# Dunni3/keypoint-diffusion

Measured on AMD Instinct MI355X. Metric: denoising steps/sec, higher is better.
Workload: dtype f32; 1 GPU; egnn_all_atom dynamics (6 EGNN layers, hidden 256, update_kp_feat; fixed receptor encoder), batch of 64 synthetic 300-atom pockets / 25-atom ligands per GPU, T=500, seeded random-init weights, every step taken from the t=T ligand state; batch_per_gpu=64, n_rec=300, n_lig=25, parallelism=dp1

## Files before the change

keypoint-diffusion_amd/csrc/egnn.hip:

```cpp
#include <string.h>

#include <map>
#include <set>
#include <string>
#include <vector>

#include "egnn_kernels.h"
#include "egnn_wide.h"
#include "mfma_core.h"

using namespace kpd;

namespace {

struct LayerW {
    float *wp_e[4], *wx_e[4], *b_e[4], *wr_e[4], *watt[4];
    float *wp_c[4], *wx_c[4], *b_c[4], *wr_c[4], *w3[4];
    void *wh_e[4], *wh_c[4];
    void *chh_p[2][NSLOT];
    void *wh_a[2], *wh_b[2], *wh_2[2];
    float *wp_p[2][NSLOT], *wx_p[2][NSLOT], *b_p[2][NSLOT];
    float *ch_p[2][NSLOT], *wcol_p[2][NSLOT];
    float *wp_a[2], *wx_a[2], *wp_b[2], *wx_b[2], *b0[2], *wp_2[2], *wx_2[2], *b2[2], *ln_w[2], *ln_b[2];
};
// ... 517 lines not shown
                                       void *stream) {
    KPD_REQUIRE(m && bt && t_dev && eps_h && eps_x, KPD_ERR_INVALID, "null argument");
    KPD_REQUIRE(m->wide || m->committed, KPD_ERR_STATE, "kpd_egnn_forward before kpd_egnn_commit");
    KPD_REQUIRE(bt->B >= 1 && bt->n_lig >= 1 && bt->n_kp >= 1, KPD_ERR_INVALID, "empty batch (B=%d n_lig=%d n_kp=%d)", bt->B, bt->n_lig, bt->n_kp);
    KPD_REQUIRE(!m->cfg.update_kp_feat || bt->n_kk == 0 || (bt->kk_src && bt->kk_dst), KPD_ERR_INVALID, "kk edges missing");
    KPD_REQUIRE(bt->kk_rowptr, KPD_ERR_INVALID, "kk_rowptr missing");
    if (m->wide) return wide_forward(m->wide, bt, t_dev, eps_h, eps_x, static_cast<hipStream_t>(stream));
    KPD_REQUIRE(bt->B <= m->cap_B && bt->n_lig <= m->cap_lig && bt->n_kp <= m->cap_kp && bt->n_kk <= m->cap_kk &&
                    bt->max_lig <= m->cap_maxlig && bt->max_kp <= m->cap_maxkp,
                KPD_ERR_CAPACITY, "batch (B=%d lig=%d kp=%d kk=%d maxlig=%d maxkp=%d) exceeds reserved workspace (%d %d %d %d %d %d)",
                bt->B, bt->n_lig, bt->n_kp, bt->n_kk, bt->max_lig, bt->max_kp, m->cap_B, m->cap_lig, m->cap_kp, m->cap_kk,
                m->cap_maxlig, m->cap_maxkp);
    hipStream_t st = static_cast<hipStream_t>(stream);
    const kpd_egnn_config &c = m->cfg;

    KPD_HIP(hipMemcpyAsync(m->x[NT_LIG], bt->lig_x, (size_t)bt->n_lig * 12, hipMemcpyDeviceToDevice, st));
    KPD_HIP(hipMemcpyAsync(m->x[NT_KP], bt->kp_x, (size_t)bt->n_kp * 12, hipMemcpyDeviceToDevice, st));
    KPD_TRY(launch_node_graph_index(bt->lig_ptr, bt->B, bt->n_lig, m->bidx[NT_LIG], st));
    KPD_TRY(launch_node_graph_index(bt->kp_ptr, bt->B, bt->n_kp, m->bidx[NT_KP], st));
    KPD_TRY(launch_lig_graph(bt, c.ll_cutoff, c.ll_k, c.kl_cutoff, c.kl_k, &m->lg, m->ll_deg, m->ll_off, m->kl_off, m->kl_pg, st));
    const int tr = TM;
    const int active = c.update_kp_feat ? 0xF : 0x3;
    const bool prune = c.update_kp_feat && m->prune_last;
    const int active_last = prune ? 0x3 : active;
    KPD_TRY(launch_egnn_meta(m->lg.counts, bt->n_kk, active, active_last, bt->lig_ptr, bt->kp_ptr, m->lg.ll_per_graph,
                             bt->kk_rowptr, bt->B, m->kl_off, c.message_norm, c.update_kp_feat, m->meta, m->z[NT_LIG],
                             m->z[NT_KP], st, tr));
    KPD_TRY(launch_embed(bt->lig_h, bt->n_lig, c.atom_nf, m->le_W0, m->le_b0, 64, m->le_W1t, m->le_b1, t_dev,
                         m->bidx[NT_LIG], m->h[NT_LIG], 0, st));
    KPD_TRY(launch_embed(bt->kp_h, bt->n_kp, c.rec_nf, m->re_W0, m->re_b0, 2 * c.rec_nf, m->re_W1t, m->re_b1, t_dev,
                         m->bidx[NT_KP], m->h[NT_KP], m->rec_identity ? 1 : 0, st));
    const int n_tab = bt->B * c.rec_nf;
    const bool kp_tab = m->kp_table && m->gemm_mode == 0 && m->tab_rows > 0 && (long)bt->B * c.rec_nf <= bt->n_kp / 2;
    m->last_table = kp_tab;
    if (kp_tab) {
        KPD_REQUIRE(n_tab <= m->tab_rows, KPD_ERR_CAPACITY, "internal: %d class rows, table of %d", n_tab, m->tab_rows);
        KPD_HIP(hipMemsetD32Async(reinterpret_cast<hipDeviceptr_t>(m->kp_ok), 0x3f800000, 1, st));
        KPD_TRY(launch_kp_classify(bt->kp_h, bt->n_kp, c.rec_nf, m->bidx[NT_KP], m->rowmap, m->kp_ok, st));
        KPD_TRY(launch_embed(m->tab_in, n_tab, c.rec_nf, m->re_W0, m->re_b0, 2 * c.rec_nf, m->re_W1t, m->re_b1, t_dev, m->tab_bidx,
                             m->hT, 0, st));
    }

    const int e_kl_cap = bt->n_kp * (c.kl_k > 0 ? c.kl_k : std::min(bt->max_lig, 100));
    const int E_cap[4] = {std::max<int>((long)bt->n_lig * std::min(bt->max_lig - 1, c.ll_k > 0 ? c.ll_k : 200), 1), e_kl_cap, e_kl_cap,
                          bt->n_kk};
    int tile_cap = 0, tile_cap_last = 0;
    for (int et = 0; et < m->n_et; ++et) {
        tile_cap += cdiv(E_cap[et], tr);
        if ((active_last >> et) & 1) tile_cap_last += cdiv(E_cap[et], tr);
    }

    const int n[2] = {bt->n_lig, bt->n_kp};
    const int *esrc[4] = {m->lg.ll_src, m->lg.kl_src, m->lg.lk_src, bt->kk_src};
// ... 37 lines not shown
                    pk.n_slots[NT_LIG] = 0;
                    pk.skip_if = m->kp_ok;
                    ProjArgs &pa = pp.nt[NT_KP];
                    pa.h = m->hT; pa.n = n_tab; pa.P = m->PT;
                    KPD_TRY(launch_proj_chain(pp, st));
                    KPD_TRY(launch_proj_chain(pk, st));
                } else {
                    KPD_TRY(launch_proj_chain(pp, st));
                }
            }
        }
        EdgeArgs ea;
        memset(&ea, 0, sizeof(ea));
        const bool last = li == n_layers - 1;
        ea.meta = last ? m->meta + 16 : m->meta;
        ea.x[0] = m->x[0]; ea.x[1] = m->x[1]; ea.P[0] = m->P[0]; ea.P[1] = m->P[1];
        ea.use_tanh = c.use_tanh; ea.coords_range = c.coords_range;
        ea.tile_rows = tr;
        ea.gemm_mode = tr == TM ? m->gemm_mode : 0;
        for (int et = 0; et < 4; ++et) {
            ea.src[et] = esrc[et]; ea.dst[et] = edst[et];
            ea.src_nt[et] = kSrcNt[et]; ea.dst_nt[et] = kDstNt[et]; ea.src_slot[et] = kSrcSlot[et]; ea.dst_slot[et] = kDstSlot[et];
            ea.wr_e[et] = L.wr_e[et]; ea.wr_c[et] = L.wr_c[et];
            ea.wp_e[et] = L.wp_e[et]; ea.wx_e[et] = L.wx_e[et]; ea.b_e[et] = L.b_e[et];
            ea.wp_c[et] = L.wp_c[et]; ea.wx_c[et] = L.wx_c[et]; ea.b_c[et] = L.b_c[et];
            ea.wh_e[et] = L.wh_e[et]; ea.wh_c[et] = L.wh_c[et];
            ea.watt[et] = L.watt[et]; ea.w3[et] = L.w3[et];
            ea.hn_main[et] = m->hn_main[et]; ea.hn_cont[et] = m->hn_cont[et];
            ea.xn_main[et] = m->xn_main[et]; ea.xn_cont[et] = m->xn_cont[et];
        }
        if (kp_tab && li == 0) { ea.PT = m->PT; ea.rowmap = m->rowmap; ea.kp_ok = m->kp_ok; }
// ... 18 lines not shown
            na.wp_a = L.wp_a[nt]; na.wx_a = L.wx_a[nt]; na.wp_b = L.wp_b[nt]; na.wx_b = L.wx_b[nt]; na.b0 = L.b0[nt];
            na.wp_2 = L.wp_2[nt]; na.wx_2 = L.wx_2[nt]; na.b2 = L.b2[nt]; na.ln_w = L.ln_w[nt]; na.ln_b = L.ln_b[nt];
            na.ln_inv_n = 1.0f / (float)(c.hidden_nf + 1); na.ln_pad = (float)(HID - c.hidden_nf);
            na.wh_a = L.wh_a[nt]; na.wh_b = L.wh_b[nt]; na.wh_2 = L.wh_2[nt];
            na.norm = c.norm;
            na.tile_shift = 6;
        };
        {
            NodeLayerPair lp;
            memset(&lp, 0, sizeof(lp));
            for (int nt = 0; nt < 2; ++nt) {
                NodeLayerArgs &na = lp.nt[nt];
                na.u.n = n[nt]; na.u.h = m->h[nt];
                if (nt < m->n_upd && !(nt == NT_KP && last && prune)) {
                    fill_update(na.u, nt);
                    na.do_update = 1;
                }
                if (!na.do_update && !na.do_proj) na.u.n = 0;
            }
            lp.tiles0 = cdiv(lp.nt[0].u.n, TN);
            lp.gemm_mode = m->gemm_mode;
            KPD_TRY(launch_node_layer(lp, st));
        }
    }
    KPD_TRY(launch_decode(m->h[NT_LIG], m->x[NT_LIG], bt->lig_x, bt->n_lig, c.atom_nf, 2 * c.atom_nf, m->de_W0, m->de_b0,
                          m->de_W1, m->de_b1, eps_h, eps_x, st));
    return KPD_OK;
}

extern "C" kpd_status kpd_egnn_debug_state(kpd_egnn *m, const char *what, float *out, int64_t n_floats, void *stream) {
    KPD_REQUIRE(m && what && out, KPD_ERR_INVALID, "null argument");
    hipStream_t st = static_cast<hipStream_t>(stream);
    if (m->wide) return wide_debug_state(m->wide, what, out, n_floats, st);
    const std::string w(what);
    const float *src = nullptr;
    if (w == "h_lig") src = m->h[0];
    else if (w == "h_kp") src = m->h[1];
    else if (w == "x_lig") src = m->x[0];
    else if (w == "x_kp") src = m->x[1];
// ... 100 lines not shown
```

keypoint-diffusion_amd/csrc/egnn_kernels.h:

```cpp
#pragma once
#include "engine.h"

namespace kpd {

constexpr int NSLOT = 8;
constexpr int ATT_BIAS_AT = 260;
constexpr int BIAS_K = 260;
constexpr int ET_LL = 0, ET_KL = 1, ET_LK = 2, ET_KK = 3;
constexpr int NT_LIG = 0, NT_KP = 1;

constexpr int EDGE_LDS_BYTES = TM * SA * 4 + (TM * 2 + TM + 3 * TM + TM + 3 * TM + 4 * HS + 8 + TM) * 4;
constexpr int EDGE_KPT_LDS_BYTES = EDGE_LDS_BYTES + 2 * TM * 4;
constexpr int EDGE_H_LDS_BYTES = 64 * 280 * 2 * 2 + (TM * 2 + TM + 3 * TM + TM + 3 * TM + 2 * HS + 8) * 4 + 2 * 2 * 272 * 2;

struct ProjArgs {
    const float *h;
    int n;
    float *P;
    const float *wp[NSLOT];
    const float *wx[NSLOT];
    const float *bias[NSLOT];
    int slot[NSLOT];
    const float *chain[NSLOT];
    const float *wcol[NSLOT];
    const void *chain_h[NSLOT];
};

// ... 70 lines not shown
    float *att[4], *sc[4], *nvec[4];
    const float *dij[4];
    const float *wa[4], *w3[4];
    const float *wpT[4][2], *wxT[4][2], *wr[4][2];
    float *dv_main[4][2], *dv_cont[4][2], *dvw_main[4][2], *dvw_cont[4][2];
    float *part[2];
    int part_ld;
    int use_tanh;
    float coords_range;
};

struct NodeArgs {
    int n;
    float *h;
    float *x;
    const int *bidx;
    const float *z;
    int n_in;
    const int *rowptr[2];
    const float *hn_main[2], *hn_cont[2];
    const float *xn_main[2], *xn_cont[2];
    const float *wp_a, *wx_a, *wp_b, *wx_b, *b0;
    const float *wp_2, *wx_2, *b2;
    const void *wh_a, *wh_b, *wh_2;
    const float *ln_w, *ln_b;
    int norm;
    float ln_inv_n, ln_pad;
    int tile_shift;
};

// ... 7 lines not shown
};

struct NodeLayerPair {
    NodeLayerArgs nt[2];
    int tiles0;
    int gemm_mode;
};

constexpr int TN = 32;
constexpr int NODE_LAYER_LDS_BYTES = TN * SA * 4 + 3 * TN * 4 + 3 * HS * 4;
constexpr int NODE_H_TILE_FLOATS = 2 * TN * 280 / 2;
constexpr int NODE_H_LDS_BYTES = NODE_H_TILE_FLOATS * 4 + 3 * TN * 4;


kpd_status egnn_kernels_init();
kpd_status launch_node_graph_index(const int *ptr, int B, int n, int *bidx, hipStream_t st);
kpd_status launch_egnn_meta(const int *counts, int e_kk, int active_mask, int active_last, const int *lig_ptr, const int *kp_ptr,
                            const int *ll_per_graph, const int *kk_rowptr, int B, const int *kl_off, float message_norm,
                            int update_kp, int *meta, float *z_lig, float *z_kp, hipStream_t st, int tile_rows = TM);
kpd_status launch_embed(const float *in, int n, int fin, const float *W0, const float *b0, int hid, const float *W1t,
                        const float *b1, const float *t, const int *bidx, float *out, int identity, hipStream_t st);
kpd_status launch_kp_classify(const float *kp_h, int n, int fin, const int *bidx, int *rowmap, int *ok, hipStream_t st);
kpd_status launch_decode(const float *h, const float *x, const float *x0, int n, int atom_nf, int hid, const float *W0,
                         const float *b0, const float *W1, const float *b1, float *eps_h, float *eps_x, hipStream_t st);
kpd_status launch_egnn_edge(const EdgeArgs &a, int tile_cap, hipStream_t st);
kpd_status launch_egnn_edge_train(const EdgeTrainArgs &a, int tile_cap, hipStream_t st);
struct EdgePiecesSumArgs {
    const float *hn_main[4], *hn_cont[4], *xn_main[4], *xn_cont[4];
    const int *rowptr[4];
    int live[4], dst_nt[4];
    const float *zinv[2];
    int n[2];
    float *hn[2], *xn[2];
};
kpd_status launch_edge_pieces_sum(const EdgePiecesSumArgs &a, hipStream_t st);
kpd_status launch_edge_train_pack(const EdgePackTab &t, hipStream_t st);
kpd_status launch_egnn_edge_bwd(const EdgeBwdArgs &a, int tile_cap, hipStream_t st);
// ... 15 lines not shown
```

keypoint-diffusion_amd/csrc/egnn_kernels.hip:

```cpp
#include <stdlib.h>

#include <algorithm>

#include "egnn_kernels.h"
#include "mfma_core.h"

namespace kpd {

__global__ void k_node_graph_index(const int *__restrict__ ptr, int B, int n, int *__restrict__ bidx) {
    const int i = blockIdx.x * blockDim.x + threadIdx.x;
    if (i >= n) return;
    int lo = 0, hi = B;
    while (hi - lo > 1) {
        const int mid = (lo + hi) >> 1;
        if (ptr[mid] <= i) lo = mid; else hi = mid;
    }
    bidx[i] = lo;
}

__global__ void k_kp_classify(const float *__restrict__ kp_h, int n, int fin, const int *__restrict__ bidx, int *__restrict__ rowmap,
                              int *__restrict__ ok) {
    const int v = blockIdx.x * blockDim.x + threadIdx.x;
    if (v >= n) return;
    const unsigned *row = reinterpret_cast<const unsigned *>(kp_h) + (size_t)v * fin;
    int ones = 0, other = 0, c = 0;
    for (int k = 0; k < fin; ++k) {
        const unsigned u = row[k];
        if (u == 0x3f800000u) { ++ones; c = k; }
        else if (u != 0u) other = 1;
    }
    rowmap[v] = bidx[v] * fin + c;
    if (ones != 1 || other) *ok = 0;
}

__global__ void k_egnn_meta(const int *__restrict__ counts, int e_kk, int active_mask, int active_last, const int *__restrict__ lig_ptr,
                            const int *__restrict__ kp_ptr, const int *__restrict__ ll_per_graph,
                            const int *__restrict__ kk_rowptr, int B, const int *__restrict__ kl_off, float message_norm,
                            int update_kp, int tile_rows, int *__restrict__ meta, float *__restrict__ z_lig, float *__restrict__ z_kp) {
    if (blockIdx.x == 0 && threadIdx.x < 2) {
        const int mask = threadIdx.x ? active_last : active_mask;
        int *mt = meta + 16 * threadIdx.x;
        int E[4] = {counts[0], counts[1], counts[1], e_kk};
        int run = 0;
        for (int et = 0; et < 4; ++et) {
            if (!((mask >> et) & 1)) E[et] = 0;
            mt[et] = E[et];
            mt[4 + et] = run;
// ... 109 lines not shown
    }
    if (lane < 3) eps_x[(size_t)v * 3 + lane] = x[(size_t)v * 3 + lane] - x0[(size_t)v * 3 + lane];
}

constexpr unsigned PROW_B = NSLOT * HS * 4;

struct EdgeSmem {
    float *A;
    int *src, *dst;
    int *gsrc, *gdst;
    float *d, *xd, *att, *mx;
    float *wv;
    int *misc;
};

template <bool KPT = false>
__device__ __forceinline__ EdgeSmem edge_smem(float *smem) {
    EdgeSmem s;
    s.A = smem;
    s.src = reinterpret_cast<int *>(smem + TM * SA);
    s.dst = s.src + TM;
    s.d = reinterpret_cast<float *>(s.dst + TM);
    s.xd = s.d + TM;
    s.att = s.xd + 3 * TM;
    s.mx = s.att + TM;
    s.wv = s.mx + 3 * TM;
    s.misc = reinterpret_cast<int *>(s.wv + 4 * HS);
    s.gsrc = KPT ? s.misc + 8 + TM : s.src;
    s.gdst = KPT ? s.gsrc + TM : s.dst;
    return s;
}

template <int NW>
struct EdgeGather {
    static constexpr int RPW = TM / NW;
    f32x4 ps[RPW], pd[RPW];
    f32x4 tps, tpd;
};

template <int NW>
__device__ __forceinline__ void edge_gather_issue(EdgeGather<NW> &g, const EdgeSmem &s, const float *__restrict__ Ps,
                                                  const float *__restrict__ Pd, int wave, int lane) {
    constexpr int RPW = TM / NW;
    const char *ps = reinterpret_cast<const char *>(Ps), *pd = reinterpret_cast<const char *>(Pd);
// ... 23 lines not shown
#pragma unroll
    for (int rr = 0; rr < RPW; ++rr) {
        const unsigned ou = (unsigned)__builtin_amdgcn_readlane(iu, rr) * PROW_B, ov = (unsigned)__builtin_amdgcn_readlane(iv, rr) * PROW_B;
        g.ps[rr] = *reinterpret_cast<const f32x4 *>(ps + (ou + 16u * lane));
        g.pd[rr] = *reinterpret_cast<const f32x4 *>(pd + (ov + 16u * lane));
    }
    const unsigned ou = (unsigned)__shfl(iu, (lane >> 2) & (RPW - 1)) * PROW_B, ov = (unsigned)__shfl(iv, (lane >> 2) & (RPW - 1)) * PROW_B;
    if (lane < 4 * RPW && (lane & 3) < 2) {
        const int c = lane & 3;
        g.tps = *reinterpret_cast<const f32x4 *>(ps + (ou + 16u * (64 + c)));
        g.tpd = *reinterpret_cast<const f32x4 *>(pd + (ov + 16u * (64 + c)));
    }
}

template <int NW>
__device__ __forceinline__ void edge_gather_finish(const EdgeGather<NW> &g, const EdgeSmem &s, const float *__restrict__ wr, int wave,
                                                   int lane) {
    constexpr int RPW = TM / NW;
    const f32x4 w0 = reinterpret_cast<const f32x4 *>(wr)[lane];
    f32x4 dv[(RPW + 3) / 4];
#pragma unroll
    for (int i = 0; i < (RPW + 3) / 4; ++i) dv[i] = *reinterpret_cast<const f32x4 *>(s.d + wave * RPW + 4 * i);
#pragma unroll
    for (int rr = 0; rr < RPW; ++rr) {
        const int r = wave * RPW + rr;
        f32x4 v = g.ps[rr] + g.pd[rr] + dv[rr >> 2][rr & 3] * w0;
        v = silu_pre4(v);
        *reinterpret_cast<f32x4 *>(s.A + r * SA + 4 * lane) = v;
    }
    if (lane < 4 * RPW && (lane & 3) < 2) {
// ... 32 lines not shown
                    for (int i = 0; i < 4; ++i) T[acc_row(mt, r4 + i, lane) * SA + col] = y[i];
                }
            } else {
#pragma unroll
                for (int reg = 0; reg < 16; ++reg) T[acc_row(mt, reg, lane) * SA + col] = silu(acc[mt][nt][reg] + bb);
            }
        }
    }
    if ((tid % TPR) == 0) T[(tid / TPR) * SA + 256] = PRE ? silu_pre(ex) : silu(ex + b[256]);
}

template <int NW, bool KPT>
__device__ __forceinline__ void egnn_edge_tile(const EdgeArgs &a) {
    constexpr int TPR = NW;
    extern __shared__ __attribute__((aligned(16))) float smem[];
    const EdgeSmem s = edge_smem<KPT>(smem);
    const int tid = threadIdx.x, wave = tid >> 6, lane = tid & 63;
    const int T = a.meta[8];
    const int chunk = (T + 7) >> 3;
    const int bi = blockIdx.x >> 3;
    int tl = bi, bsel = 3;
    const int rem = a.split_slots > 0 ? chunk % a.split_slots : 0;
    if (rem > 0 && 2 * rem <= a.split_slots) {
        const int full = chunk - rem;
        if (bi >= full) {
            const int j = bi - full;
            if (j >= 2 * rem) return;
            tl = full + (j >> 1);
            bsel = 1 << (j & 1);
        }
    } else if (bi >= chunk) return;
    const int tile = (blockIdx.x & 7) * chunk + tl;
// ... 7 lines not shown
    const int ne = min(TM, a.meta[et] - e0);
    const int snt = a.src_nt[et], dnt = a.dst_nt[et];
    const int *__restrict__ esrc = a.src[et];
    const int *__restrict__ edst = a.dst[et];

    const float *Ps = a.P[snt] + (size_t)a.src_slot[et] * HS;
    const float *Pd = a.P[dnt] + (size_t)a.dst_slot[et] * HS;
    [[maybe_unused]] const int *maps = nullptr, *mapd = nullptr;
    if constexpr (KPT) {
        if (*a.kp_ok) {
            if (snt == NT_KP) { maps = a.rowmap; Ps = a.PT + (size_t)a.src_slot[et] * HS; }
            if (dnt == NT_KP) { mapd = a.rowmap; Pd = a.PT + (size_t)a.dst_slot[et] * HS; }
        }
    }
    EdgeGather<NW> ge;
    if constexpr (KPT) {
        if (bsel & 1) edge_gather_issue_early<NW>(ge, esrc, edst, e0, ne, Ps, Pd, wave, lane, maps, mapd);
    } else {
        if (bsel & 1) edge_gather_issue_early<NW>(ge, esrc, edst, e0, ne, Ps, Pd, wave, lane);
    }
    __builtin_amdgcn_sched_barrier(0);
    if (tid < TM) {
        const int e = e0 + min(tid, ne - 1);
        const int u = esrc[e], v = edst[e];
        s.src[tid] = (int)((unsigned)u * PROW_B);
        s.dst[tid] = (int)((unsigned)v * PROW_B);
        if constexpr (KPT) {
            s.gsrc[tid] = (int)((unsigned)(maps ? maps[u] : u) * PROW_B);
            s.gdst[tid] = (int)((unsigned)(mapd ? mapd[v] : v) * PROW_B);
        }
        const float *xs = a.x[snt] + (size_t)u * 3, *xd = a.x[dnt] + (size_t)v * 3;
        const float dx = xs[0] - xd[0], dy = xs[1] - xd[1], dz = xs[2] - xd[2];
        const float d = sqrtf(dx * dx + dy * dy + dz * dz);
        const float inv = 1.0f / (d + 1.0f);
        s.d[tid] = d;
        s.xd[3 * tid] = dx * inv;
        s.xd[3 * tid + 1] = dy * inv;
        s.xd[3 * tid + 2] = dz * inv;
        const int vprev = tid > 0 ? edst[e0 + min(tid - 1, ne - 1)] : (e0 > 0 ? edst[e0 - 1] : -1);
        const int vnext = tid + 1 < ne ? edst[e0 + tid + 1] : -2;
        const unsigned long long heads = __ballot(tid < ne && (tid == 0 || vprev != v));
        const unsigned long long ends = __ballot(tid < ne && vnext != v);
        if (tid == 0) {
            s.misc[0] = (vprev == v) ? 1 : 0;
            s.misc[2] = (int)(ends & 0xffffffffu);
            s.misc[3] = (int)(ends >> 32);
            s.misc[4] = (int)(heads & 0xffffffffu);
            s.misc[5] = (int)(heads >> 32);
        }
    } else {
        for (int i = tid - TM; i < 4 * 66; i += 64 * NW - TM) {
            const int which = i / 66, j = i - which * 66;
            const float *row = which == 0 ? a.watt[et] : which == 1 ? a.w3[et] : which == 2 ? a.wx_e[et] : a.wx_c[et];
            reinterpret_cast<f32x4 *>(s.wv + which * HS)[j] = reinterpret_cast<const f32x4 *>(row)[j];
        }
    }
    [[maybe_unused]] BPrefetch bpre;
    if constexpr (NW == 4) gemm_b_prefetch(bpre, (bsel & 1) ? a.wp_e[et] : a.wp_c[et], wave, lane);
    lds_barrier();

    const int first_is_cont = s.misc[0];
    const unsigned long long endmask =
        ((unsigned long long)(unsigned)s.misc[3] << 32) | (unsigned long long)(unsigned)s.misc[2];
    f32x16 acc[2][WaveCols<NW>::NT];
    float ex;
    EdgeGather<NW == 4 ? 4 : TM> gc;

    if (bsel & 1) {
    edge_gather_finish<NW>(ge, s, a.wr_e[et], wave, lane);
    lds_barrier();
    acc_zero_w<NW>(acc);
    ex = row_dot_chunks<TPR>(s.A, s.wv + 2 * HS, KP / 4, tid);
    if constexpr (NW == 4) gemm_rows64_pre<NG, SA>(s.A, a.wp_e[et], acc, wave, lane, bpre);
    else gemm_rows64_w<NW, NG, SA>(s.A, a.wp_e[et], acc, wave, lane);
    if constexpr (NW == 4) gemm_b_prefetch(bpre, a.wp_c[et], wave, lane);
    lds_barrier();
    store_T_silu_w<NW, true>(s.A, acc, ex, a.b_e[et], tid, wave, lane);
    if constexpr (NW == 4) {
        if (bsel & 2) {
            edge_gather_issue<NW>(gc, s, Ps + HS, Pd + HS, wave, lane);
            __builtin_amdgcn_sched_barrier(0);
        }
    }
    lds_barrier();
    float dot = row_dot_chunks<TPR>(s.A, s.wv, 64, tid);
    const int row = tid / TPR;
    if ((tid % TPR) == 0) {
        dot = fmaf(s.A[row * SA + 256], s.wv[256], dot);
        s.att[row] = row < ne ? sigmoidf_(dot + s.wv[ATT_BIAS_AT]) * (1.0f / SILU_C) : 0.0f;
    }
    lds_barrier();
    float *hmain = a.hn_main[et], *hcont = a.hn_cont[et] + (size_t)tile_in_et * HS;
    if (tid < 256) {
        float run = 0.0f;
        int piece = 0;
#pragma unroll 1
        for (int r0 = 0; r0 < TM; r0 += 16) {
            if (r0 >= ne) break;
            float v[16], w[16];
            int dvv[16];
            {
                typedef int i32x4 __attribute__((ext_vector_type(4)));
#pragma unroll
                for (int j = 0; j < 4; ++j) {
                    const i32x4 t = *reinterpret_cast<const i32x4 *>(s.dst + r0 + 4 * j);
                    dvv[4 * j] = t[0]; dvv[4 * j + 1] = t[1]; dvv[4 * j + 2] = t[2]; dvv[4 * j + 3] = t[3];
                }
            }
#pragma unroll
            for (int i = 0; i < 16; ++i) {
                w[i] = s.att[r0 + i];
                v[i] = s.A[(r0 + i) * SA + tid];
            }
#pragma unroll
            for (int i = 0; i < 16; ++i) {
                run = fmaf(v[i], w[i], run);
                if ((endmask >> (r0 + i)) & 1ull) {
                    float *out = (piece == 0 && first_is_cont) ? hcont : hmain + ((unsigned)dvv[i] / (unsigned)(NSLOT * 4));
                    out[tid] = run;
                    run = 0.0f;
                    ++piece;
                }
            }
        }
    }
    if (wave == NW - 1) reinterpret_cast<float *>(s.misc + 8)[lane] = s.A[lane * SA + 256] * s.att[lane];
    lds_barrier();
    }

    if (bsel & 2) {
    if constexpr (NW == 4) {
        if (!(bsel & 1)) edge_gather_issue<NW>(gc, s, Ps + HS, Pd + HS, wave, lane);
        edge_gather_finish<NW>(gc, s, a.wr_c[et], wave, lane);
    } else build_edge_A<NW>(s, Ps + HS, Pd + HS, a.wr_c[et], wave, lane);
    lds_barrier();
    acc_zero_w<NW>(acc);
    ex = row_dot_chunks<TPR>(s.A, s.wv + 3 * HS, KP / 4, tid);
    if constexpr (NW == 4) gemm_rows64_pre<NG, SA>(s.A, a.wp_c[et], acc, wave, lane, bpre);
    else gemm_rows64_w<NW, NG, SA>(s.A, a.wp_c[et], acc, wave, lane);
    lds_barrier();
    store_T_silu_w<NW, true>(s.A, acc, ex, a.b_c[et], tid, wave, lane);
    lds_barrier();
    float dot = row_dot_chunks<TPR>(s.A, s.wv + HS, 64, tid);
    const int row = tid / TPR;
    if ((tid % TPR) == 0) {
        dot = fmaf(s.A[row * SA + 256], s.wv[HS + 256], dot);
        float c = a.use_tanh ? tanhf(dot) * a.coords_range : dot;
// ... 1039 lines not shown
                if (hi0 > lo0) {
                    sx += m0x; sy += m0y; sz += m0z;
                    for (int t = (lo0 >> a.tile_shift) + 1; t <= ((hi0 - 1) >> a.tile_shift); ++t) {
                        const float *q = a.xn_cont[0] + (size_t)t * 4;
                        sx += q[0]; sy += q[1]; sz += q[2];
                    }
                }
                if (hi1 > lo1) {
                    sx += m1x; sy += m1y; sz += m1z;
                    for (int t = (lo1 >> a.tile_shift) + 1; t <= ((hi1 - 1) >> a.tile_shift); ++t) {
                        const float *q = a.xn_cont[two] + (size_t)t * 4;
                        sx += q[0]; sy += q[1]; sz += q[2];
                    }
                }
                float *xv = a.x + (size_t)v * 3;
                xv[0] += sx / z; xv[1] += sy / z; xv[2] += sz / z;
            }
            s_z[tid] = z;
        } else if (tid >= 512 - 3 * 66) {
            const int i = tid - (512 - 3 * 66), which = i / 66, j = i - which * 66;
            const float *row = which == 0 ? a.wx_a : which == 1 ? a.wx_b : a.wx_2;
            reinterpret_cast<f32x4 *>(s_wx + which * HS)[j] = reinterpret_cast<const f32x4 *>(row)[j];
        }
        load_h();
        lds_barrier();
#pragma unroll
        for (int i = 0; i < 16; ++i) acc[i] = 0.0f;
        gemm_rows32_t8<NG, SA>(A, a.wp_a, acc, wave, lane);
        float ex = row_dot_chunks<TPR>(A, s_wx, KP / 4, tid);
        lds_barrier();
        {
// ... 180 lines not shown
        if (v < a.n) {
            z = a.z[a.bidx[v]];
            float sx = 0.f, sy = 0.f, sz = 0.f;
            for (int i = 0; i < a.n_in; ++i) {
                const int lo = a.rowptr[i][v], hi = a.rowptr[i][v + 1];
                if (hi > lo) {
                    const float *pm = a.xn_main[i] + (size_t)v * 4;
                    sx += pm[0]; sy += pm[1]; sz += pm[2];
                    for (int t = (lo >> a.tile_shift) + 1; t <= ((hi - 1) >> a.tile_shift); ++t) {
                        const float *q = a.xn_cont[i] + (size_t)t * 4;
                        sx += q[0]; sy += q[1]; sz += q[2];
                    }
                }
            }
            float *xv = a.x + (size_t)v * 3;
            xv[0] += sx / z; xv[1] += sy / z; xv[2] += sz / z;
        }
        s_z[tid] = z;
    }
#pragma unroll
    for (int rr = 0; rr < RPW; ++rr) {
        const int r = wave * RPW + rr, v = node0 + r;
        f32x4 val = {0.f, 0.f, 0.f, 0.f}, val2 = {0.f, 0.f, 0.f, 0.f};
        if (v < a.n) {
            const f32x4 *src = reinterpret_cast<const f32x4 *>(a.h + (size_t)v * HS);
            val = src[lane];
            if (lane < 2) val2 = src[64 + lane];
        }
        put_row(r, val, val2);
    }
    lds_barrier();
// ... 95 lines not shown
            const float mean = s_mean[r], rstd = s_rstd[r];
            const f32x4 w = reinterpret_cast<const f32x4 *>(a.ln_w)[lane];
            const f32x4 b = reinterpret_cast<const f32x4 *>(a.ln_b)[lane];
            val = (val - mean) * rstd * w + b;
            last = (last - mean) * rstd * a.ln_w[256] + a.ln_b[256];
        }
        f32x4 *dst = reinterpret_cast<f32x4 *>(a.h + (size_t)v * HS);
        dst[lane] = val;
        if (lane == 0) dst[64] = f32x4{last, 0.f, 0.f, 0.f};
    }
}


kpd_status egnn_kernels_init() { return KPD_OK; }

kpd_status launch_node_graph_index(const int *ptr, int B, int n, int *bidx, hipStream_t st) {
    if (n == 0) return KPD_OK;
    hipLaunchKernelGGL(k_node_graph_index, dim3(cdiv(n, 256)), dim3(256), 0, st, ptr, B, n, bidx);
    KPD_LAUNCH_CHECK();
    return KPD_OK;
}

kpd_status launch_egnn_meta(const int *counts, int e_kk, int active_mask, int active_last, const int *lig_ptr, const int *kp_ptr,
                            const int *ll_per_graph, const int *kk_rowptr, int B, const int *kl_off, float message_norm,
                            int update_kp, int *meta, float *z_lig, float *z_kp, hipStream_t st, int tile_rows) {
    hipLaunchKernelGGL(k_egnn_meta, dim3(cdiv(B, 256)), dim3(256), 0, st, counts, e_kk, active_mask, active_last, lig_ptr, kp_ptr,
                       ll_per_graph, kk_rowptr, B, kl_off, message_norm, update_kp, tile_rows, meta, z_lig, z_kp);
    KPD_LAUNCH_CHECK();
    return KPD_OK;
}

kpd_status launch_embed(const float *in, int n, int fin, const float *W0, const float *b0, int hid, const float *W1t,
                        const float *b1, const float *t, const int *bidx, float *out, int identity, hipStream_t st) {
    if (n == 0) return KPD_OK;
    KPD_REQUIRE(fin <= 256 && hid <= 512, KPD_ERR_INVALID, "embed: fin=%d hid=%d exceed 256 / 512", fin, hid);
    if (hid <= 256 || identity)
        hipLaunchKernelGGL(k_embed<256>, dim3(cdiv(n, EMB_NODES)), dim3(256), 0, st, in, n, fin, W0, b0, hid, W1t, b1, t, bidx,
                           out, identity);
    else
        hipLaunchKernelGGL(k_embed<512>, dim3(cdiv(n, EMB_NODES)), dim3(256), 0, st, in, n, fin, W0, b0, hid, W1t, b1, t, bidx,
                           out, identity);
    KPD_LAUNCH_CHECK();
    return KPD_OK;
}

kpd_status launch_kp_classify(const float *kp_h, int n, int fin, const int *bidx, int *rowmap, int *ok, hipStream_t st) {
    if (n == 0) return KPD_OK;
    hipLaunchKernelGGL(k_kp_classify, dim3(cdiv(n, 256)), dim3(256), 0, st, kp_h, n, fin, bidx, rowmap, ok);
    KPD_LAUNCH_CHECK();
    return KPD_OK;
}

kpd_status launch_decode(const float *h, const float *x, const float *x0, int n, int atom_nf, int hid, const float *W0,
                         const float *b0, const float *W1, const float *b1, float *eps_h, float *eps_x,
                         hipStream_t st) {
    if (n == 0) return KPD_OK;
    KPD_REQUIRE(hid <= 512 && atom_nf <= 256, KPD_ERR_INVALID, "decode: hid=%d atom_nf=%d exceed 512 / 256", hid, atom_nf);
    if (hid <= 64 && atom_nf <= 64)
        hipLaunchKernelGGL(k_decode<64>, dim3(n), dim3(64), 0, st, h, x, x0, n, atom_nf, hid, W0, b0, W1, b1, eps_h, eps_x);
    else
        hipLaunchKernelGGL(k_decode<512>, dim3(n), dim3(64), 0, st, h, x, x0, n, atom_nf, hid, W0, b0, W1, b1, eps_h, eps_x);
    KPD_LAUNCH_CHECK();
    return KPD_OK;
}

kpd_status launch_egnn_edge(const EdgeArgs &a, int tile_cap, hipStream_t st) {
    if (tile_cap == 0) return KPD_OK;
    if (poison_level() >= 1) KPD_TRY(poison_lds(st));
    KPD_REQUIRE(a.tile_rows == TM, KPD_ERR_INVALID, "the edge kernels walk 64-edge tiles");
    if (a.gemm_mode == 1) {
        for (int et = 0; et < 4; ++et)
            KPD_REQUIRE(!a.wp_e[et] || (a.wh_e[et] && a.wh_c[et]), KPD_ERR_STATE, "f16x2 weights of edge type %d were not packed", et);
        KPD_TRY(ensure_dynamic_lds(reinterpret_cast<const void *>(k_egnn_edge_h<4>), EDGE_H_LDS_BYTES));
        hipLaunchKernelGGL(k_egnn_edge_h<4>, dim3(8 * cdiv(tile_cap, 8)), dim3(256), EDGE_H_LDS_BYTES, st, a);
        KPD_LAUNCH_CHECK();
        return KPD_OK;
    }
    EdgeArgs b = a;
    b.split_slots = 2 * cu_count() / 8;
    if (a.kp_ok) {
        KPD_REQUIRE(a.PT && a.rowmap, KPD_ERR_INVALID, "edge launch: keypoint class table without its rows or row map");
        KPD_TRY(ensure_dynamic_lds(reinterpret_cast<const void *>(k_egnn_edge_kpt), EDGE_KPT_LDS_BYTES));
        hipLaunchKernelGGL(k_egnn_edge_kpt, dim3(8 * (cdiv(tile_cap, 8) + b.split_slots / 2)), dim3(256), EDGE_KPT_LDS_BYTES, st, b);
        KPD_LAUNCH_CHECK();
        return KPD_OK;
    }
    KPD_TRY(ensure_dynamic_lds(reinterpret_cast<const void *>(k_egnn_edge<4>), EDGE_LDS_BYTES));
    hipLaunchKernelGGL(k_egnn_edge<4>, dim3(8 * (cdiv(tile_cap, 8) + b.split_slots / 2)), dim3(256), EDGE_LDS_BYTES, st, b);
    KPD_LAUNCH_CHECK();
    return KPD_OK;
}

kpd_status launch_node_layer(const NodeLayerPair &p, hipStream_t st) {
    const int tiles = p.tiles0 + cdiv(p.nt[1].u.n, TN);
    if (tiles == 0) return KPD_OK;
    if (poison_level() >= 1) KPD_TRY(poison_lds(st));
    for (int nt = 0; nt < 2; ++nt)
        KPD_REQUIRE(p.nt[nt].u.n == 0 || (p.nt[nt].do_update && !p.nt[nt].do_proj), KPD_ERR_INVALID, "node launch: update-only node types expected");
// ... 67 lines not shown
```

keypoint-diffusion_amd/csrc/mfma_core.h:

```cpp
#pragma once
#include "common.h"

namespace kpd {

typedef float f32x16 __attribute__((ext_vector_type(16)));
typedef float f32x4 __attribute__((ext_vector_type(4)));

__device__ __forceinline__ float silu(float x) { return x * __builtin_amdgcn_rcpf(1.0f + __expf(-x)); }
constexpr float SILU_C = -1.4426950408889634f;
__device__ __forceinline__ float silu_pre(float xs) { return xs * __builtin_amdgcn_rcpf(1.0f + __builtin_amdgcn_exp2f(xs)); }
typedef float silu_f32x4 __attribute__((ext_vector_type(4)));
__device__ __forceinline__ silu_f32x4 silu_pre4(silu_f32x4 v) {
    const silu_f32x4 q = {__builtin_amdgcn_rcpf(1.0f + __builtin_amdgcn_exp2f(v[0])), __builtin_amdgcn_rcpf(1.0f + __builtin_amdgcn_exp2f(v[1])),
                          __builtin_amdgcn_rcpf(1.0f + __builtin_amdgcn_exp2f(v[2])), __builtin_amdgcn_rcpf(1.0f + __builtin_amdgcn_exp2f(v[3]))};
    return v * q;
}
__device__ __forceinline__ float sigmoidf_(float x) { return __builtin_amdgcn_rcpf(1.0f + __expf(-x)); }

__device__ __forceinline__ void acc_zero(f32x16 (&acc)[2][2]) {
#pragma unroll
    for (int m = 0; m < 2; ++m)
#pragma unroll
        for (int n = 0; n < 2; ++n)
#pragma unroll
// ... 476 lines not shown
            s = fmaf((float)hi[4 + j] + (float)lo[4 + j], w1[j], s);
        }
    }
#pragma unroll
    for (int o = 1; o < TPR; o <<= 1) s += __shfl_xor(s, o);
    return s;
}

__device__ __forceinline__ float silu_pre_x64(float xs) {
    return xs * __builtin_amdgcn_rcpf(fmaf(__builtin_amdgcn_exp2f(xs), 1.0f / H_SCALE_A, 1.0f / H_SCALE_A));
}

template <int TPR>
__device__ __forceinline__ float row_dot_chunks(const float *__restrict__ T, const float *__restrict__ w, int chunks, int tid) {
    const int row = tid / TPR, q = tid % TPR;
    const f32x4 *a = reinterpret_cast<const f32x4 *>(T + row * SA);
    const f32x4 *wv = reinterpret_cast<const f32x4 *>(w);
    float s = 0.0f;
#pragma unroll
    for (int i = 0; i < (66 + TPR - 1) / TPR; ++i) {
        const int c = q + TPR * i;
        if (c < chunks) {
            const f32x4 av = a[c], wq = wv[c];
            s = fmaf(av[0], wq[0], s);
            s = fmaf(av[1], wq[1], s);
            s = fmaf(av[2], wq[2], s);
            s = fmaf(av[3], wq[3], s);
        }
    }
#pragma unroll
    for (int o = 1; o < TPR; o <<= 1) s += __shfl_xor(s, o);
    return s;
}

__device__ __forceinline__ void lds_barrier() {
    asm volatile("s_waitcnt lgkmcnt(0)\n\ts_barrier" ::: "memory");
}

// ... 7 lines not shown
```

Before: 155.5 steps/s.

## Fuse keypoint classify into graph-index kernel, drop coord copies, scalarize edge gathers

Merges the keypoint one-hot classification and the kp_ok reset into the node graph-index kernel, removing a memset and a kernel launch. Coordinates are no longer copied into the workspace up front. Layers read the input coordinates directly, and the first node update writes workspace x from them. The edge kernel precomputes row offsets once and reuses them for both gathers, using scalar base addresses, readfirstlane on wave-uniform values, and readlane for destination offsets. This also drops the extra LDS the KPT variant used. Several small per-step overheads are targeted, at the cost of more complex state tracking for which buffer holds the current coordinates.

New measurement: 157.3 steps/s, median of 6. +1.1%, better.

```diff
diff --git a/keypoint-diffusion_amd/csrc/egnn.hip b/keypoint-diffusion_amd/csrc/egnn.hip
--- a/keypoint-diffusion_amd/csrc/egnn.hip
+++ b/keypoint-diffusion_amd/csrc/egnn.hip
@@ -555,10 +555,15 @@
     hipStream_t st = static_cast<hipStream_t>(stream);
     const kpd_egnn_config &c = m->cfg;
 
-    KPD_HIP(hipMemcpyAsync(m->x[NT_LIG], bt->lig_x, (size_t)bt->n_lig * 12, hipMemcpyDeviceToDevice, st));
-    KPD_HIP(hipMemcpyAsync(m->x[NT_KP], bt->kp_x, (size_t)bt->n_kp * 12, hipMemcpyDeviceToDevice, st));
-    KPD_TRY(launch_node_graph_index(bt->lig_ptr, bt->B, bt->n_lig, m->bidx[NT_LIG], st));
-    KPD_TRY(launch_node_graph_index(bt->kp_ptr, bt->B, bt->n_kp, m->bidx[NT_KP], st));
+    const int n_tab = bt->B * c.rec_nf;
+    const bool kp_tab = m->kp_table && m->gemm_mode == 0 && m->tab_rows > 0 && (long)bt->B * c.rec_nf <= bt->n_kp / 2;
+    m->last_table = kp_tab;
+    KPD_TRY(launch_node_graph_index(bt->lig_ptr, bt->B, bt->n_lig, m->bidx[NT_LIG], st, kp_tab ? m->kp_ok : nullptr));
+    if (kp_tab)
+        KPD_TRY(launch_node_graph_index(bt->kp_ptr, bt->B, bt->n_kp, m->bidx[NT_KP], st, nullptr, bt->kp_h, c.rec_nf, m->rowmap, m->kp_ok));
+    else
+        KPD_TRY(launch_node_graph_index(bt->kp_ptr, bt->B, bt->n_kp, m->bidx[NT_KP], st));
+    const float *x_cur[2] = {bt->lig_x, bt->kp_x};
     KPD_TRY(launch_lig_graph(bt, c.ll_cutoff, c.ll_k, c.kl_cutoff, c.kl_k, &m->lg, m->ll_deg, m->ll_off, m->kl_off, m->kl_pg, st));
     const int tr = TM;
     const int active = c.update_kp_feat ? 0xF : 0x3;
@@ -571,13 +576,8 @@
                          m->bidx[NT_LIG], m->h[NT_LIG], 0, st));
     KPD_TRY(launch_embed(bt->kp_h, bt->n_kp, c.rec_nf, m->re_W0, m->re_b0, 2 * c.rec_nf, m->re_W1t, m->re_b1, t_dev,
                          m->bidx[NT_KP], m->h[NT_KP], m->rec_identity ? 1 : 0, st));
-    const int n_tab = bt->B * c.rec_nf;
-    const bool kp_tab = m->kp_table && m->gemm_mode == 0 && m->tab_rows > 0 && (long)bt->B * c.rec_nf <= bt->n_kp / 2;
-    m->last_table = kp_tab;
     if (kp_tab) {
         KPD_REQUIRE(n_tab <= m->tab_rows, KPD_ERR_CAPACITY, "internal: %d class rows, table of %d", n_tab, m->tab_rows);
-        KPD_HIP(hipMemsetD32Async(reinterpret_cast<hipDeviceptr_t>(m->kp_ok), 0x3f800000, 1, st));
-        KPD_TRY(launch_kp_classify(bt->kp_h, bt->n_kp, c.rec_nf, m->bidx[NT_KP], m->rowmap, m->kp_ok, st));
         KPD_TRY(launch_embed(m->tab_in, n_tab, c.rec_nf, m->re_W0, m->re_b0, 2 * c.rec_nf, m->re_W1t, m->re_b1, t_dev, m->tab_bidx,
                              m->hT, 0, st));
     }
@@ -645,7 +645,7 @@
         memset(&ea, 0, sizeof(ea));
         const bool last = li == n_layers - 1;
         ea.meta = last ? m->meta + 16 : m->meta;
-        ea.x[0] = m->x[0]; ea.x[1] = m->x[1]; ea.P[0] = m->P[0]; ea.P[1] = m->P[1];
+        ea.x[0] = x_cur[0]; ea.x[1] = x_cur[1]; ea.P[0] = m->P[0]; ea.P[1] = m->P[1];
         ea.use_tanh = c.use_tanh; ea.coords_range = c.coords_range;
         ea.tile_rows = tr;
         ea.gemm_mode = tr == TM ? m->gemm_mode : 0;
@@ -694,6 +694,7 @@
                 na.u.n = n[nt]; na.u.h = m->h[nt];
                 if (nt < m->n_upd && !(nt == NT_KP && last && prune)) {
                     fill_update(na.u, nt);
+                    na.u.x_in = x_cur[nt] == m->x[nt] ? nullptr : x_cur[nt];
                     na.do_update = 1;
                 }
                 if (!na.do_update && !na.do_proj) na.u.n = 0;
@@ -701,8 +702,12 @@
             lp.tiles0 = cdiv(lp.nt[0].u.n, TN);
             lp.gemm_mode = m->gemm_mode;
             KPD_TRY(launch_node_layer(lp, st));
-        }
-    }
+            for (int nt = 0; nt < 2; ++nt)
+                if (lp.nt[nt].do_update) x_cur[nt] = m->x[nt];
+        }
+    }
+    if (x_cur[NT_LIG] != m->x[NT_LIG]) KPD_HIP(hipMemcpyAsync(m->x[NT_LIG], bt->lig_x, (size_t)bt->n_lig * 12, hipMemcpyDeviceToDevice, st));
+    if (x_cur[NT_KP] != m->x[NT_KP]) KPD_HIP(hipMemcpyAsync(m->x[NT_KP], bt->kp_x, (size_t)bt->n_kp * 12, hipMemcpyDeviceToDevice, st));
     KPD_TRY(launch_decode(m->h[NT_LIG], m->x[NT_LIG], bt->lig_x, bt->n_lig, c.atom_nf, 2 * c.atom_nf, m->de_W0, m->de_b0,
                           m->de_W1, m->de_b1, eps_h, eps_x, st));
     return KPD_OK;
diff --git a/keypoint-diffusion_amd/csrc/egnn_kernels.h b/keypoint-diffusion_amd/csrc/egnn_kernels.h
--- a/keypoint-diffusion_amd/csrc/egnn_kernels.h
+++ b/keypoint-diffusion_amd/csrc/egnn_kernels.h
@@ -10,7 +10,6 @@
 constexpr int NT_LIG = 0, NT_KP = 1;
 
 constexpr int EDGE_LDS_BYTES = TM * SA * 4 + (TM * 2 + TM + 3 * TM + TM + 3 * TM + 4 * HS + 8 + TM) * 4;
-constexpr int EDGE_KPT_LDS_BYTES = EDGE_LDS_BYTES + 2 * TM * 4;
 constexpr int EDGE_H_LDS_BYTES = 64 * 280 * 2 * 2 + (TM * 2 + TM + 3 * TM + TM + 3 * TM + 2 * HS + 8) * 4 + 2 * 2 * 272 * 2;
 
 struct ProjArgs {
@@ -111,6 +110,7 @@
     int n;
     float *h;
     float *x;
+    const float *x_in;
     const int *bidx;
     const float *z;
     int n_in;
@@ -148,13 +148,13 @@
 
 
 kpd_status egnn_kernels_init();
-kpd_status launch_node_graph_index(const int *ptr, int B, int n, int *bidx, hipStream_t st);
+kpd_status launch_node_graph_index(const int *ptr, int B, int n, int *bidx, hipStream_t st, int *set_ok = nullptr,
+                                   const float *kp_h = nullptr, int fin = 0, int *rowmap = nullptr, int *ok = nullptr);
 kpd_status launch_egnn_meta(const int *counts, int e_kk, int active_mask, int active_last, const int *lig_ptr, const int *kp_ptr,
                             const int *ll_per_graph, const int *kk_rowptr, int B, const int *kl_off, float message_norm,
                             int update_kp, int *meta, float *z_lig, float *z_kp, hipStream_t st, int tile_rows = TM);
 kpd_status launch_embed(const float *in, int n, int fin, const float *W0, const float *b0, int hid, const float *W1t,
                         const float *b1, const float *t, const int *bidx, float *out, int identity, hipStream_t st);
-kpd_status launch_kp_classify(const float *kp_h, int n, int fin, const int *bidx, int *rowmap, int *ok, hipStream_t st);
 kpd_status launch_decode(const float *h, const float *x, const float *x0, int n, int atom_nf, int hid, const float *W0,
                          const float *b0, const float *W1, const float *b1, float *eps_h, float *eps_x, hipStream_t st);
 kpd_status launch_egnn_edge(const EdgeArgs &a, int tile_cap, hipStream_t st);
diff --git a/keypoint-diffusion_amd/csrc/egnn_kernels.hip b/keypoint-diffusion_amd/csrc/egnn_kernels.hip
--- a/keypoint-diffusion_amd/csrc/egnn_kernels.hip
+++ b/keypoint-diffusion_amd/csrc/egnn_kernels.hip
@@ -7,21 +7,8 @@
 
 namespace kpd {
 
-__global__ void k_node_graph_index(const int *__restrict__ ptr, int B, int n, int *__restrict__ bidx) {
-    const int i = blockIdx.x * blockDim.x + threadIdx.x;
-    if (i >= n) return;
-    int lo = 0, hi = B;
-    while (hi - lo > 1) {
-        const int mid = (lo + hi) >> 1;
-        if (ptr[mid] <= i) lo = mid; else hi = mid;
-    }
-    bidx[i] = lo;
-}
-
-__global__ void k_kp_classify(const float *__restrict__ kp_h, int n, int fin, const int *__restrict__ bidx, int *__restrict__ rowmap,
-                              int *__restrict__ ok) {
-    const int v = blockIdx.x * blockDim.x + threadIdx.x;
-    if (v >= n) return;
+__device__ __forceinline__ void kp_classify_row(const float *__restrict__ kp_h, int v, int graph, int fin, int *__restrict__ rowmap,
+                                                int *__restrict__ ok) {
     const unsigned *row = reinterpret_cast<const unsigned *>(kp_h) + (size_t)v * fin;
     int ones = 0, other = 0, c = 0;
     for (int k = 0; k < fin; ++k) {
@@ -29,8 +16,22 @@
         if (u == 0x3f800000u) { ++ones; c = k; }
         else if (u != 0u) other = 1;
     }
-    rowmap[v] = bidx[v] * fin + c;
+    rowmap[v] = graph * fin + c;
     if (ones != 1 || other) *ok = 0;
+}
+
+__global__ void k_node_graph_index(const int *__restrict__ ptr, int B, int n, int *__restrict__ bidx, int *__restrict__ set_ok,
+                                   const float *__restrict__ kp_h, int fin, int *__restrict__ rowmap, int *__restrict__ ok) {
+    const int i = blockIdx.x * blockDim.x + threadIdx.x;
+    if (i == 0 && set_ok) *set_ok = 0x3f800000;
+    if (i >= n) return;
+    int lo = 0, hi = B;
+    while (hi - lo > 1) {
+        const int mid = (lo + hi) >> 1;
+        if (ptr[mid] <= i) lo = mid; else hi = mid;
+    }
+    bidx[i] = lo;
+    if (kp_h) kp_classify_row(kp_h, i, lo, fin, rowmap, ok);
 }
 
 __global__ void k_egnn_meta(const int *__restrict__ counts, int e_kk, int active_mask, int active_last, const int *__restrict__ lig_ptr,
@@ -170,7 +171,6 @@
     int *misc;
 };
 
-template <bool KPT = false>
 __device__ __forceinline__ EdgeSmem edge_smem(float *smem) {
     EdgeSmem s;
     s.A = smem;
@@ -182,8 +182,8 @@
     s.mx = s.att + TM;
     s.wv = s.mx + 3 * TM;
     s.misc = reinterpret_cast<int *>(s.wv + 4 * HS);
-    s.gsrc = KPT ? s.misc + 8 + TM : s.src;
-    s.gdst = KPT ? s.gsrc + TM : s.dst;
+    s.gsrc = s.src;
+    s.gdst = s.dst;
     return s;
 }
 
@@ -237,6 +237,66 @@
 }
 
 template <int NW>
+struct EdgeRowOffs {
+    unsigned ou[TM / NW], ov[TM / NW];
+    unsigned tu, tv;
+};
+
+template <int NW>
+__device__ __forceinline__ void edge_row_offsets(EdgeRowOffs<NW> &o, const int *__restrict__ esrc, const int *__restrict__ edst, int e0, int ne,
+                                                 int wave, int lane, const int *__restrict__ maps, const int *__restrict__ mapd) {
+    constexpr int RPW = TM / NW;
+    const int *es = esrc + e0, *ed = edst + e0;
+    const int last = ne - 1;
+    int iu[RPW], iv[RPW];
+#pragma unroll
+    for (int rr = 0; rr < RPW; ++rr) {
+        const int r = min(wave * RPW + rr, last);
+        iu[rr] = es[r];
+        iv[rr] = ed[r];
+    }
+    const int rl = min(wave * RPW + ((lane >> 2) & (RPW - 1)), last);
+    int tu = es[rl], tv = ed[rl];
+    if (maps) {
+#pragma unroll
+        for (int rr = 0; rr < RPW; ++rr) iu[rr] = maps[iu[rr]];
+        tu = maps[tu];
+    }
+    if (mapd) {
+#pragma unroll
+        for (int rr = 0; rr < RPW; ++rr) iv[rr] = mapd[iv[rr]];
+        tv = mapd[tv];
+    }
+#pragma unroll
+    for (int rr = 0; rr < RPW; ++rr) {
+        o.ou[rr] = (unsigned)iu[rr] * PROW_B;
+        o.ov[rr] = (unsigned)iv[rr] * PROW_B;
+    }
+    o.tu = (unsigned)tu * PROW_B + 16u * (64 + (lane & 3));
+    o.tv = (unsigned)tv * PROW_B + 16u * (64 + (lane & 3));
+}
+
+typedef __attribute__((address_space(1))) const char gchar;
+template <int NW>
+__device__ __forceinline__ void edge_gather_issue_s(EdgeGather<NW> &g, const EdgeRowOffs<NW> &o, const float *__restrict__ Ps,
+                                                    const float *__restrict__ Pd, int lane) {
+    constexpr int RPW = TM / NW;
+    gchar *ps = (gchar *)reinterpret_cast<const char *>(Ps), *pd = (gchar *)reinterpret_cast<const char *>(Pd);
+    const unsigned vo = 16u * lane;
+#pragma unroll
+    for (int rr = 0; rr < RPW; ++rr) {
+        gchar *bs = ps + o.ou[rr], *bd = pd + o.ov[rr];
+        asm volatile("" : "+s"(bs), "+s"(bd));
+        g.ps[rr] = *reinterpret_cast<gf32x4 *>(bs + vo);
+        g.pd[rr] = *reinterpret_cast<gf32x4 *>(bd + vo);
+    }
+    if (lane < 4 * RPW && (lane & 3) < 2) {
+        g.tps = *reinterpret_cast<gf32x4 *>(ps + o.tu);
+        g.tpd = *reinterpret_cast<gf32x4 *>(pd + o.tv);
+    }
+}
+
+template <int NW>
 __device__ __forceinline__ void edge_gather_finish(const EdgeGather<NW> &g, const EdgeSmem &s, const float *__restrict__ wr, int wave,
                                                    int lane) {
     constexpr int RPW = TM / NW;
@@ -299,8 +359,8 @@
 __device__ __forceinline__ void egnn_edge_tile(const EdgeArgs &a) {
     constexpr int TPR = NW;
     extern __shared__ __attribute__((aligned(16))) float smem[];
-    const EdgeSmem s = edge_smem<KPT>(smem);
-    const int tid = threadIdx.x, wave = tid >> 6, lane = tid & 63;
+    const EdgeSmem s = edge_smem(smem);
+    const int tid = threadIdx.x, wave = __builtin_amdgcn_readfirstlane(tid >> 6), lane = tid & 63;
     const int T = a.meta[8];
     const int chunk = (T + 7) >> 3;
     const int bi = blockIdx.x >> 3;
@@ -338,8 +398,10 @@
         }
     }
     EdgeGather<NW> ge;
-    if constexpr (KPT) {
-        if (bsel & 1) edge_gather_issue_early<NW>(ge, esrc, edst, e0, ne, Ps, Pd, wave, lane, maps, mapd);
+    [[maybe_unused]] EdgeRowOffs<NW> ro;
+    if constexpr (NW == 4) {
+        edge_row_offsets<NW>(ro, esrc, edst, e0, ne, wave, lane, maps, mapd);
+        if (bsel & 1) edge_gather_issue_s<NW>(ge, ro, Ps, Pd, lane);
     } else {
         if (bsel & 1) edge_gather_issue_early<NW>(ge, esrc, edst, e0, ne, Ps, Pd, wave, lane);
     }
@@ -349,10 +411,6 @@
         const int u = esrc[e], v = edst[e];
         s.src[tid] = (int)((unsigned)u * PROW_B);
         s.dst[tid] = (int)((unsigned)v * PROW_B);
-        if constexpr (KPT) {
-            s.gsrc[tid] = (int)((unsigned)(maps ? maps[u] : u) * PROW_B);
-            s.gdst[tid] = (int)((unsigned)(mapd ? mapd[v] : v) * PROW_B);
-        }
         const float *xs = a.x[snt] + (size_t)u * 3, *xd = a.x[dnt] + (size_t)v * 3;
         const float dx = xs[0] - xd[0], dy = xs[1] - xd[1], dz = xs[2] - xd[2];
         const float d = sqrtf(dx * dx + dy * dy + dz * dz);
@@ -383,9 +441,9 @@
     if constexpr (NW == 4) gemm_b_prefetch(bpre, (bsel & 1) ? a.wp_e[et] : a.wp_c[et], wave, lane);
     lds_barrier();
 
-    const int first_is_cont = s.misc[0];
-    const unsigned long long endmask =
-        ((unsigned long long)(unsigned)s.misc[3] << 32) | (unsigned long long)(unsigned)s.misc[2];
+    const int first_is_cont = __builtin_amdgcn_readfirstlane(s.misc[0]);
+    const unsigned long long endmask = ((unsigned long long)(unsigned)__builtin_amdgcn_readfirstlane(s.misc[3]) << 32) |
+                                       (unsigned long long)(unsigned)__builtin_amdgcn_readfirstlane(s.misc[2]);
     f32x16 acc[2][WaveCols<NW>::NT];
     float ex;
     EdgeGather<NW == 4 ? 4 : TM> gc;
@@ -402,7 +460,7 @@
     store_T_silu_w<NW, true>(s.A, acc, ex, a.b_e[et], tid, wave, lane);
     if constexpr (NW == 4) {
         if (bsel & 2) {
-            edge_gather_issue<NW>(gc, s, Ps + HS, Pd + HS, wave, lane);
+            edge_gather_issue_s<NW>(gc, ro, Ps + HS, Pd + HS, lane);
             __builtin_amdgcn_sched_barrier(0);
         }
     }
@@ -418,29 +476,23 @@
     if (tid < 256) {
         float run = 0.0f;
         int piece = 0;
+        const int dall = s.dst[lane];
 #pragma unroll 1
         for (int r0 = 0; r0 < TM; r0 += 16) {
             if (r0 >= ne) break;
             float v[16], w[16];
-            int dvv[16];
-            {
-                typedef int i32x4 __attribute__((ext_vector_type(4)));
-#pragma unroll
-                for (int j = 0; j < 4; ++j) {
-                    const i32x4 t = *reinterpret_cast<const i32x4 *>(s.dst + r0 + 4 * j);
-                    dvv[4 * j] = t[0]; dvv[4 * j + 1] = t[1]; dvv[4 * j + 2] = t[2]; dvv[4 * j + 3] = t[3];
-                }
-            }
 #pragma unroll
             for (int i = 0; i < 16; ++i) {
                 w[i] = s.att[r0 + i];
                 v[i] = s.A[(r0 + i) * SA + tid];
             }
+            const unsigned ends16 = (unsigned)(endmask >> r0);
 #pragma unroll
             for (int i = 0; i < 16; ++i) {
                 run = fmaf(v[i], w[i], run);
-                if ((endmask >> (r0 + i)) & 1ull) {
-                    float *out = (piece == 0 && first_is_cont) ? hcont : hmain + ((unsigned)dvv[i] / (unsigned)(NSLOT * 4));
+                if (__builtin_expect((ends16 >> i) & 1u, 0)) {
+                    const unsigned doff = (unsigned)__builtin_amdgcn_readlane(dall, r0 + i) / (unsigned)(NSLOT * 4);
+                    float *out = (piece == 0 && first_is_cont) ? hcont : hmain + doff;
                     out[tid] = run;
                     run = 0.0f;
                     ++piece;
@@ -454,7 +506,7 @@
 
     if (bsel & 2) {
     if constexpr (NW == 4) {
-        if (!(bsel & 1)) edge_gather_issue<NW>(gc, s, Ps + HS, Pd + HS, wave, lane);
+        if (!(bsel & 1)) edge_gather_issue_s<NW>(gc, ro, Ps + HS, Pd + HS, lane);
         edge_gather_finish<NW>(gc, s, a.wr_c[et], wave, lane);
     } else build_edge_A<NW>(s, Ps + HS, Pd + HS, a.wr_c[et], wave, lane);
     lds_barrier();
@@ -1524,7 +1576,8 @@
                     }
                 }
                 float *xv = a.x + (size_t)v * 3;
-                xv[0] += sx / z; xv[1] += sy / z; xv[2] += sz / z;
+                const float *xi = (a.x_in ? a.x_in : a.x) + (size_t)v * 3;
+                xv[0] = xi[0] + sx / z; xv[1] = xi[1] + sy / z; xv[2] = xi[2] + sz / z;
             }
             s_z[tid] = z;
         } else if (tid >= 512 - 3 * 66) {
@@ -1735,7 +1788,8 @@
                 }
             }
             float *xv = a.x + (size_t)v * 3;
-            xv[0] += sx / z; xv[1] += sy / z; xv[2] += sz / z;
+            const float *xi = (a.x_in ? a.x_in : a.x) + (size_t)v * 3;
+            xv[0] = xi[0] + sx / z; xv[1] = xi[1] + sy / z; xv[2] = xi[2] + sz / z;
         }
         s_z[tid] = z;
     }
@@ -1861,9 +1915,11 @@
 
 kpd_status egnn_kernels_init() { return KPD_OK; }
 
-kpd_status launch_node_graph_index(const int *ptr, int B, int n, int *bidx, hipStream_t st) {
+kpd_status launch_node_graph_index(const int *ptr, int B, int n, int *bidx, hipStream_t st, int *set_ok, const float *kp_h, int fin,
+                                   int *rowmap, int *ok) {
     if (n == 0) return KPD_OK;
-    hipLaunchKernelGGL(k_node_graph_index, dim3(cdiv(n, 256)), dim3(256), 0, st, ptr, B, n, bidx);
+    KPD_REQUIRE(!kp_h || (fin > 0 && rowmap && ok), KPD_ERR_INVALID, "node graph index: one-hot test without its outputs");
+    hipLaunchKernelGGL(k_node_graph_index, dim3(cdiv(n, 256)), dim3(256), 0, st, ptr, B, n, bidx, set_ok, kp_h, fin, rowmap, ok);
     KPD_LAUNCH_CHECK();
     return KPD_OK;
 }
@@ -1891,13 +1947,6 @@
     return KPD_OK;
 }
 
-kpd_status launch_kp_classify(const float *kp_h, int n, int fin, const int *bidx, int *rowmap, int *ok, hipStream_t st) {
-    if (n == 0) return KPD_OK;
-    hipLaunchKernelGGL(k_kp_classify, dim3(cdiv(n, 256)), dim3(256), 0, st, kp_h, n, fin, bidx, rowmap, ok);
-    KPD_LAUNCH_CHECK();
-    return KPD_OK;
-}
-
 kpd_status launch_decode(const float *h, const float *x, const float *x0, int n, int atom_nf, int hid, const float *W0,
                          const float *b0, const float *W1, const float *b1, float *eps_h, float *eps_x,
                          hipStream_t st) {
@@ -1927,8 +1976,8 @@
     b.split_slots = 2 * cu_count() / 8;
     if (a.kp_ok) {
         KPD_REQUIRE(a.PT && a.rowmap, KPD_ERR_INVALID, "edge launch: keypoint class table without its rows or row map");
-        KPD_TRY(ensure_dynamic_lds(reinterpret_cast<const void *>(k_egnn_edge_kpt), EDGE_KPT_LDS_BYTES));
-        hipLaunchKernelGGL(k_egnn_edge_kpt, dim3(8 * (cdiv(tile_cap, 8) + b.split_slots / 2)), dim3(256), EDGE_KPT_LDS_BYTES, st, b);
+        KPD_TRY(ensure_dynamic_lds(reinterpret_cast<const void *>(k_egnn_edge_kpt), EDGE_LDS_BYTES));
+        hipLaunchKernelGGL(k_egnn_edge_kpt, dim3(8 * (cdiv(tile_cap, 8) + b.split_slots / 2)), dim3(256), EDGE_LDS_BYTES, st, b);
         KPD_LAUNCH_CHECK();
         return KPD_OK;
     }
diff --git a/keypoint-diffusion_amd/csrc/mfma_core.h b/keypoint-diffusion_amd/csrc/mfma_core.h
--- a/keypoint-diffusion_amd/csrc/mfma_core.h
+++ b/keypoint-diffusion_amd/csrc/mfma_core.h
@@ -514,14 +514,14 @@
 template <int TPR>
 __device__ __forceinline__ float row_dot_chunks(const float *__restrict__ T, const float *__restrict__ w, int chunks, int tid) {
     const int row = tid / TPR, q = tid % TPR;
-    const f32x4 *a = reinterpret_cast<const f32x4 *>(T + row * SA);
-    const f32x4 *wv = reinterpret_cast<const f32x4 *>(w);
+    const f32x4 *a = reinterpret_cast<const f32x4 *>(T + row * SA) + q;
+    const f32x4 *wv = reinterpret_cast<const f32x4 *>(w) + q;
     float s = 0.0f;
 #pragma unroll
     for (int i = 0; i < (66 + TPR - 1) / TPR; ++i) {
         const int c = q + TPR * i;
         if (c < chunks) {
-            const f32x4 av = a[c], wq = wv[c];
+            const f32x4 av = a[TPR * i], wq = wv[TPR * i];
             s = fmaf(av[0], wq[0], s);
             s = fmaf(av[1], wq[1], s);
             s = fmaf(av[2], wq[2], s);
```
